# elasticdeeplearning/trainingjob-operator

Measured on AMD Instinct MI355X. Metric: tokens_per_sec_llama3_8b, higher is better.
Workload: dtype bf16; 1 GPU; model=llama3-8b, global_batch=4, seq_len=4096, parallelism=dp1, micro_batch=2, grad_accum=2, checkpoint_activations=False

## Files before the change

trainingjob_operator_amd/ops/hip/attention.hip:

```cpp

#include <hip/hip_runtime.h>
#include <hip/hip_bf16.h>
#include <cstdint>
#include <cstdlib>
#include <cstring>

typedef unsigned short u16;
typedef unsigned int u32;
typedef __attribute__((ext_vector_type(8))) __bf16 bf16x8;
typedef __attribute__((ext_vector_type(4))) float f32x4;

#define ATTN_BM 64
#define ATTN_BN 64
#define ATTN_D 128
#define ATTN_WAVES 4
__device__ __forceinline__ u16 attn_f2bf(float f) {
  __hip_bfloat16_raw r = __float2bfloat16(f);
  return r.x;
}

__device__ __forceinline__ float bf2f_(u16 b) {
  union { u32 u; float f; } c;
  c.u = ((u32)b) << 16;
  return c.f;
}

__device__ __forceinline__ int k_byte(int row, int col_elem) {
  return (row * ATTN_D * 2 + col_elem * 2) ^ ((row & 15) << 4);
}

#define VT_PITCH_B 144
__device__ __forceinline__ int vt_byte(int d, int kv) {
  const int m = d >> 3;
  return (d * VT_PITCH_B + kv * 2) ^
         ((((m & 7) | (((m >> 1) & 1) << 3))) << 4);
}

__device__ __forceinline__ int p_byte(int row, int col_elem) {
  return (row * ATTN_BN * 2 + col_elem * 2) ^ ((row & 7) << 4);
}


#define ATTN_SCHED_LEGACY 0
#define ATTN_SCHED_BALANCED 1

struct AttnBlock { int rank, head, batch; };

__host__ __device__ __forceinline__ AttnBlock attn_sched_block(
    unsigned id, unsigned n_row_blocks, unsigned n_heads, unsigned batch,
    int sched) {
  AttnBlock blk;
  if (sched == ATTN_SCHED_LEGACY) {
    const unsigned t = id / n_row_blocks;
    blk.rank = (int)(id - t * n_row_blocks);
    blk.batch = (int)(t / n_heads);
    blk.head = (int)(t - (unsigned)blk.batch * n_heads);
    return blk;
  }
  const unsigned M = n_heads * batch;
  const unsigned r = id / M;
  const unsigned w = id - r * M;
  const unsigned p = (M % 8 == 0) ? (w % 8) * (M / 8) + w / 8 : w;
  blk.rank = (int)r;
  blk.batch = (int)(p / n_heads);
  blk.head = (int)(p - (unsigned)blk.batch * n_heads);
  return blk;
}


#define ATTN_STRIPS_IDENTITY 0
#define ATTN_STRIPS_FOLD 1

struct AttnStrips { int kv0w, qt0; };

__host__ __device__ __forceinline__ AttnStrips attn_bwd_strips(
    int fold, int rank, int wid, int n_row_blocks) {
  AttnStrips s;
  if (fold == ATTN_STRIPS_IDENTITY) {
    s.kv0w = rank * 256 + wid * 32;
    s.qt0 = rank * 4;
    return s;
  }
  const int half = wid < 4 ? rank : 2 * n_row_blocks - 1 - rank;
  s.kv0w = half * 128 + (wid & 3) * 32;
  s.qt0 = rank * 2;
  return s;
}

__global__ __launch_bounds__(256) void attn_fwd_kernel(
    const u16* __restrict__ q, const u16* __restrict__ k,
    const u16* __restrict__ v, u16* __restrict__ out,
    float* __restrict__ lse,
    long q_sb, long q_sh, long q_ss,
    long k_sb, long k_sh, long k_ss,
    long v_sb, long v_sh, long v_ss,
    int n_heads, int S, float scale) {
  const int qb = blockIdx.x;
  const int h = blockIdx.y;
  const int b = blockIdx.z;
  const int wid = threadIdx.x >> 6;
  const int lane = threadIdx.x & 63;
  const int low = lane & 15;
  const int kg = lane >> 4;

  __shared__ u16 ldsK[ATTN_BN * ATTN_D];
  __shared__ u16 ldsV[ATTN_D * (VT_PITCH_B / 2) + 128];
  __shared__ u16 ldsP[ATTN_WAVES][16 * ATTN_BN];

  const u16* qbase = q + (long)b * q_sb + (long)h * q_sh
                     + (long)(qb * ATTN_BM) * q_ss;
  union { bf16x8 v; uint4 u; } qfrag[4];
#pragma unroll
  for (int ks = 0; ks < 4; ++ks) {
    qfrag[ks].u = *reinterpret_cast<const uint4*>(
        qbase + (long)(wid * 16 + low) * q_ss + ks * 32 + kg * 8);
  }

  float m_run[4], l_run[4];
  float oacc[8][4];
#pragma unroll
  for (int r = 0; r < 4; ++r) { m_run[r] = -INFINITY; l_run[r] = 0.f; }
#pragma unroll
  for (int ct = 0; ct < 8; ++ct)
#pragma unroll
    for (int r = 0; r < 4; ++r) oacc[ct][r] = 0.f;

  const u16* kbase = k + (long)b * k_sb + (long)h * k_sh;
  const u16* vbase = v + (long)b * v_sb + (long)h * v_sh;
  const int kv_end = (qb + 1) * ATTN_BM;
  char* ldsKb = reinterpret_cast<char*>(ldsK);
  char* ldsVb = reinterpret_cast<char*>(ldsV);
  char* ldsPb = reinterpret_cast<char*>(ldsP[wid]);

  for (int kv0 = 0; kv0 < kv_end; kv0 += ATTN_BN) {
#pragma unroll
    for (int t = 0; t < 4; ++t) {
      const int idx = t * 256 + threadIdx.x;
      const int r = idx >> 4;
      const int c8 = (idx & 15) * 8;
      *reinterpret_cast<uint4*>(&ldsKb[k_byte(r, c8)]) =
          *reinterpret_cast<const uint4*>(
              kbase + (long)(kv0 + r) * k_ss + c8);
      union { uint4 u; u16 h[8]; } vv;
      vv.u = *reinterpret_cast<const uint4*>(
          vbase + (long)(kv0 + r) * v_ss + c8);
#pragma unroll
      for (int j = 0; j < 8; ++j)
        *reinterpret_cast<u16*>(&ldsVb[vt_byte(c8 + j, r)]) = vv.h[j];
    }
    __syncthreads();

    f32x4 sacc[4];
#pragma unroll
    for (int ct = 0; ct < 4; ++ct) {
      f32x4 acc = {0.f, 0.f, 0.f, 0.f};
#pragma unroll
      for (int ks = 0; ks < 4; ++ks) {
        bf16x8 bfrag = *reinterpret_cast<const bf16x8*>(
            &ldsKb[k_byte(ct * 16 + low, ks * 32 + kg * 8)]);
        acc = __builtin_amdgcn_mfma_f32_16x16x32_bf16(qfrag[ks].v, bfrag,
                                                      acc, 0, 0, 0);
      }
      sacc[ct] = acc;
    }

    const int qrow0 = qb * ATTN_BM + wid * 16 + kg * 4;
    float mx[4], alpha[4], psum[4];
#pragma unroll
    for (int r = 0; r < 4; ++r) {
      mx[r] = -INFINITY;
#pragma unroll
      for (int ct = 0; ct < 4; ++ct) {
        const int col = kv0 + ct * 16 + low;
        float s = sacc[ct][r] * scale;
        if (col > qrow0 + r) s = -INFINITY;
        sacc[ct][r] = s;
        mx[r] = fmaxf(mx[r], s);
      }
#pragma unroll
      for (int off = 1; off < 16; off <<= 1)
        mx[r] = fmaxf(mx[r], __shfl_xor(mx[r], off, 64));
      const float mnew = fmaxf(m_run[r], mx[r]);
      alpha[r] = (m_run[r] == -INFINITY) ? 0.f : __expf(m_run[r] - mnew);
      m_run[r] = mnew;
      psum[r] = 0.f;
#pragma unroll
      for (int ct = 0; ct < 4; ++ct) {
        const float p = (sacc[ct][r] == -INFINITY)
                            ? 0.f : __expf(sacc[ct][r] - mnew);
        sacc[ct][r] = p;
        psum[r] += p;
        *reinterpret_cast<u16*>(
            &ldsPb[p_byte(kg * 4 + r, ct * 16 + low)]) = attn_f2bf(p);
      }
#pragma unroll
      for (int off = 1; off < 16; off <<= 1)
        psum[r] += __shfl_xor(psum[r], off, 64);
      l_run[r] = l_run[r] * alpha[r] + psum[r];
#pragma unroll
      for (int ct2 = 0; ct2 < 8; ++ct2) oacc[ct2][r] *= alpha[r];
    }
    __syncthreads();

#pragma unroll
    for (int ct2 = 0; ct2 < 8; ++ct2) {
      f32x4 acc = {oacc[ct2][0], oacc[ct2][1], oacc[ct2][2], oacc[ct2][3]};
#pragma unroll
      for (int ks2 = 0; ks2 < 2; ++ks2) {
        bf16x8 afrag = *reinterpret_cast<const bf16x8*>(
            &ldsPb[p_byte(low, ks2 * 32 + kg * 8)]);
        bf16x8 bfrag = *reinterpret_cast<const bf16x8*>(
            &ldsVb[vt_byte(ct2 * 16 + low, ks2 * 32 + kg * 8)]);
        acc = __builtin_amdgcn_mfma_f32_16x16x32_bf16(afrag, bfrag, acc,
                                                      0, 0, 0);
      }
#pragma unroll
      for (int r = 0; r < 4; ++r) oacc[ct2][r] = acc[r];
    }
    __syncthreads();
  }

  u16* obase = out + (((long)b * n_heads + h) * S + qb * ATTN_BM
                      + wid * 16) * ATTN_D;
#pragma unroll
  for (int r = 0; r < 4; ++r) {
    const float inv_l = 1.0f / l_run[r];
#pragma unroll
    for (int ct2 = 0; ct2 < 8; ++ct2) {
      obase[(long)(kg * 4 + r) * ATTN_D + ct2 * 16 + low] =
          attn_f2bf(oacc[ct2][r] * inv_l);
    }
  }
  if (low == 0) {
    float* lbase = lse + ((long)b * n_heads + h) * S + qb * ATTN_BM
                   + wid * 16 + kg * 4;
#pragma unroll
    for (int r = 0; r < 4; ++r) lbase[r] = m_run[r] + __logf(l_run[r]);
  }
}
// ... 1003 lines not shown
        qgp[i] += qstep;                                                    \
        __builtin_amdgcn_global_load_lds(                                   \
            (const u32*)dgp[i],                                             \
            (u32*)&lds[BUFI][DOOFF / 2 + (i * 512 + wu64 * 64) * 8],        \
            16, 0, 0);                                                      \
        dgp[i] += dostep;                                                   \
      }                                                                     \
      qtst[0] = *reinterpret_cast<const uint4*>(qtp[0]);                    \
      qtst[1] = *reinterpret_cast<const uint4*>(qtp[1]);                    \
      qtp[0] += qstep;                                                      \
      qtp[1] += qstep;                                                      \
      if (tid < 64)                                                         \
        *reinterpret_cast<float*>(&lds[BUFI][LSEOFF / 2 + tid * 2]) =       \
            lbase[(QT) * 64 + tid] * 1.4426950408889634f;                   \
      else if (tid < 128)                                                   \
        *reinterpret_cast<float*>(                                          \
            &lds[BUFI][DLTOFF / 2 + (tid - 64) * 2]) =                      \
            dbase[(QT) * 64 + tid - 64];                                    \
    }
#define BK_WRITE_QT(BUF)                                                    \
    {                                                                       \
      const int rp2_ = (tid >> 4) * 2;                                      \
      const int c8_ = (tid & 15) * 8;                                       \
      union { uint4 u4; u16 h[8]; } va_, vb_;                               \
      va_.u4 = qtst[0];                                                     \
      vb_.u4 = qtst[1];                                                     \
      _Pragma("unroll")                                                     \
      for (int j = 0; j < 8; ++j) {                                         \
        const u32 pair_ = (u32)va_.h[j] | ((u32)vb_.h[j] << 16);            \
        *reinterpret_cast<u32*>(&(BUF)[QTOFF + vt_byte(c8_ + j, rp2_)]) =   \
            pair_;                                                          \
      }                                                                     \
    }

    BK_STAGE_IN(0, qt0)
    BK_WRITE_QT(lds0)
    __syncthreads();

    int cur = 0;
    for (int qt = qt0; qt < qtn; ++qt) {
      const bool have_next = (qt + 1) < qtn;
      if (have_next) BK_STAGE_IN(cur ^ 1, qt + 1)

      char* qb_ = cur ? lds1 : lds0;
      char* dob = qb_ + DOOFF;
      char* qtb = qb_ + QTOFF;
      const float* lse2t = reinterpret_cast<const float*>(qb_ + LSEOFF);
      const float* dltt = reinterpret_cast<const float*>(qb_ + DLTOFF);
      const bool active = !CAUSAL || qt * 64 + 63 >= kv0w;
      const bool need_mask = CAUSAL && qt * 64 < kv0w + 32;

      union PF { bf16x8 v; unsigned u[4]; } pf[4];
      if (active) {
#pragma unroll
        for (int sub = 0; sub < 2; ++sub) {
          f32x16 s, dp;
#pragma unroll
          for (int r = 0; r < 16; ++r) { s[r] = 0.f; dp[r] = 0.f; }
#pragma unroll
          for (int kc = 0; kc < 8; ++kc) {
            bf16x8 a = *reinterpret_cast<const bf16x8*>(
                &qb_[k_byte(sub * 32 + low, kc * 16 + hi * 8)]);
            s = __builtin_amdgcn_mfma_f32_32x32x16_bf16(a, kf[kc].v, s,
                                                        0, 0, 0);
            bf16x8 a2 = *reinterpret_cast<const bf16x8*>(
                &dob[k_byte(sub * 32 + low, kc * 16 + hi * 8)]);
            dp = __builtin_amdgcn_mfma_f32_32x32x16_bf16(a2, vf[kc].v, dp,
                                                         0, 0, 0);
          }
#pragma unroll
          for (int r = 0; r < 16; ++r) {
            const int qr = (r & 3) + 8 * (r >> 2) + 4 * hi;
            float x = s[r] * scale2 - lse2t[sub * 32 + qr];
            if (need_mask && qt * 64 + sub * 32 + qr < kvrow) x = -1e30f;
            const float p = exp2_raw(x);
            s[r] = p * (dp[r] - dltt[sub * 32 + qr]) * scale;
          }
#pragma unroll
          for (int cc = 0; cc < 2; ++cc) {
            const int pb = cc * 8;
            unsigned a0 = cvt_pk_bf16(s[pb + 0], s[pb + 1]);
            unsigned b0 = cvt_pk_bf16(s[pb + 4], s[pb + 5]);
            unsigned a1 = cvt_pk_bf16(s[pb + 2], s[pb + 3]);
            unsigned b1 = cvt_pk_bf16(s[pb + 6], s[pb + 7]);
            auto r02 = __builtin_amdgcn_permlane32_swap(a0, b0, false, false);
            auto r13 = __builtin_amdgcn_permlane32_swap(a1, b1, false, false);
            PF f;
            f.u[0] = r02[0];
            f.u[1] = r13[0];
            f.u[2] = r02[1];
            f.u[3] = r13[1];
            pf[sub * 2 + cc] = f;
          }
        }
      }
      if (have_next) {
        char* nb = cur ? lds0 : lds1;
        BK_WRITE_QT(nb)
      }
      if (active) {
#pragma unroll
        for (int c = 0; c < 4; ++c) {
#pragma unroll
          for (int ds = 0; ds < 4; ++ds) {
            bf16x8 af = *reinterpret_cast<const bf16x8*>(
                &qtb[vt_byte(ds * 32 + low, c * 16 + hi * 8)]);
            dkacc[ds] = __builtin_amdgcn_mfma_f32_32x32x16_bf16(
                af, pf[c].v, dkacc[ds], 0, 0, 0);
          }
        }
      }
      __syncthreads();
      cur ^= 1;
    }
  }

  if (SPLIT) {
    float* wrow =
        ws + (((long)b * n_heads + blk.head) * S_kv + kvrow) * ATTN_D;
#pragma unroll
    for (int ds = 0; ds < 4; ++ds) {
#pragma unroll
      for (int g = 0; g < 4; ++g) {
        const int d0 = 8 * g + 4 * hi + 32 * ds;
        float4 wv;
        wv.x = dkacc[ds][4 * g + 0];
        wv.y = dkacc[ds][4 * g + 1];
        wv.z = dkacc[ds][4 * g + 2];
        wv.w = dkacc[ds][4 * g + 3];
        *reinterpret_cast<float4*>(wrow + d0) = wv;
      }
    }
    return;
  }
  u16* dkrow = dk + (long)b * dk_sb + (long)hkv * dk_sh + (long)kvrow * dk_ss;
#pragma unroll
  for (int ds = 0; ds < 4; ++ds) {
#pragma unroll
    for (int g = 0; g < 4; ++g) {
      const int d0 = 8 * g + 4 * hi + 32 * ds;
      const unsigned w0 = cvt_pk_bf16(dkacc[ds][4 * g + 0],
                                      dkacc[ds][4 * g + 1]);
      const unsigned w1 = cvt_pk_bf16(dkacc[ds][4 * g + 2],
                                      dkacc[ds][4 * g + 3]);
      uint2 wv;
      wv.x = w0;
      wv.y = w1;
      *reinterpret_cast<uint2*>(dkrow + d0) = wv;
    }
  }
}




struct AttnStride { long sb, sh, ss; };

static inline AttnStride attn_dense_stride(int n_heads, int S) {
  return {(long)n_heads * S * ATTN_D, (long)S * ATTN_D, (long)ATTN_D};
}

static void launch_delta(hipStream_t st, const void* out, const void* dout,
                         void* delta, AttnStride os, AttnStride dos,
                         int batch, int n_heads, int S) {
  hipLaunchKernelGGL(attn_delta_kernel, dim3(S / 16, n_heads, batch),
                     dim3(256), 0, st,
                     (const u16*)dout, (const u16*)out, (float*)delta,
                     dos.sb, dos.sh, dos.ss, os.sb, os.sh, os.ss,
                     n_heads, S);
}


__global__ __launch_bounds__(256) void attn_bwd_reduce_kernel(
    const float* __restrict__ ws_k, const float* __restrict__ ws_v,
    u16* __restrict__ dk, u16* __restrict__ dv,
    long dk_sb, long dk_sh, long dk_ss,
    long dv_sb, long dv_sh, long dv_ss,
    int n_heads, int n_kv_heads, int S, long n_rows) {
  const long row = (long)blockIdx.x * 16 + (threadIdx.x >> 4);
  if (row >= n_rows) return;
  const int sub = threadIdx.x & 15;
  const int gqa_group = n_heads / n_kv_heads;
  const long bh = row / S;
  const int s = (int)(row - bh * S);
  const long bi = bh / n_kv_heads;
  const int hkv = (int)(bh - bi * n_kv_heads);
  const bool is_v = blockIdx.y != 0;
  const float* src = (is_v ? ws_v : ws_k)
      + ((bi * n_heads + (long)hkv * gqa_group) * S + s) * ATTN_D + sub * 8;
  const long hstep = (long)S * ATTN_D;
  float4 a0 = reinterpret_cast<const float4*>(src)[0];
  float4 a1 = reinterpret_cast<const float4*>(src)[1];
  for (int g = 1; g < gqa_group; ++g) {
    const float4 p0 = reinterpret_cast<const float4*>(src + g * hstep)[0];
    const float4 p1 = reinterpret_cast<const float4*>(src + g * hstep)[1];
    a0.x += p0.x; a0.y += p0.y; a0.z += p0.z; a0.w += p0.w;
    a1.x += p1.x; a1.y += p1.y; a1.z += p1.z; a1.w += p1.w;
  }
  uint4 o;
  o.x = cvt_pk_bf16(a0.x, a0.y);
  o.y = cvt_pk_bf16(a0.z, a0.w);
  o.z = cvt_pk_bf16(a1.x, a1.y);
  o.w = cvt_pk_bf16(a1.z, a1.w);
  u16* dst = is_v
      ? dv + bi * dv_sb + (long)hkv * dv_sh + (long)s * dv_ss
      : dk + bi * dk_sb + (long)hkv * dk_sh + (long)s * dk_ss;
  *reinterpret_cast<uint4*>(dst + sub * 8) = o;
}

static inline bool attn_block_shape_ok(int batch, int n_heads,
                                       int n_kv_heads, int S) {
  return S > 0 && S % 256 == 0 && n_heads > 0 && batch > 0 &&
         n_kv_heads > 0 && n_heads % n_kv_heads == 0 &&
         attn_grid_ok(S, n_heads, batch);
}

#define ATTN_NUM_CUS 256
static bool attn_bwd_use_split(int batch, int n_heads, int n_kv_heads, int S,
                               bool causal) {
  const char* e = std::getenv("AITJ_ATTN_BWD_SPLIT");
  if (e && std::strcmp(e, "1") == 0) return true;
  if (!e || std::strcmp(e, "auto") != 0) return false;
  if (n_heads == n_kv_heads) return false;
  const long wgs = (long)batch * n_kv_heads * (S / 256);
  return wgs < (long)(causal ? 2 : 1) * ATTN_NUM_CUS;
}

static int attn_bwd_use_fold(int batch, int n_heads, int n_kv_heads, int S,
                             bool causal, bool split) {
  if (!causal) return ATTN_STRIPS_IDENTITY;
  const char* e = std::getenv("AITJ_ATTN_BWD_FOLD");
  if (e && std::strcmp(e, "0") == 0) return ATTN_STRIPS_IDENTITY;
  if (e && std::strcmp(e, "1") == 0) return ATTN_STRIPS_FOLD;
  const long wgs = (long)batch * (split ? n_heads : n_kv_heads) * (S / 256);
  return wgs <= ATTN_NUM_CUS ? ATTN_STRIPS_FOLD : ATTN_STRIPS_IDENTITY;
}

extern "C" int attn_bwd_strips_decode(int fold, int rank, int wid,
                                      int n_row_blocks, int* kv0w, int* qt0) {
  if (n_row_blocks <= 0 || rank < 0 || rank >= n_row_blocks || wid < 0 ||
      wid >= 8 || (fold != ATTN_STRIPS_IDENTITY && fold != ATTN_STRIPS_FOLD))
    return -1;
  const AttnStrips s = attn_bwd_strips(fold, rank, wid, n_row_blocks);
  *kv0w = s.kv0w;
  *qt0 = s.qt0;
  return 0;
}

extern "C" long attn_bwd_ws_bytes(int batch, int n_heads, int n_kv_heads,
                                  int S, int causal) {
  if (!attn_block_shape_ok(batch, n_heads, n_kv_heads, S)) return 0;
  if (!attn_bwd_use_split(batch, n_heads, n_kv_heads, S, causal != 0))
    return 0;
  return 2L * batch * n_heads * S * ATTN_D * (long)sizeof(float);
}

static inline bool attn_rect_shape_ok(int batch, int n_heads, int n_kv_heads,
                                      int S_q, int S_kv, bool causal) {
  return attn_block_shape_ok(batch, n_heads, n_kv_heads, S_q) &&
         attn_block_shape_ok(batch, n_heads, n_kv_heads, S_kv) &&
         !(causal && S_q != S_kv);
}

extern "C" long attn_bwd_ws_bytes_rect(int batch, int n_heads, int n_kv_heads,
                                       int S_q, int S_kv, int causal) {
  if (!attn_rect_shape_ok(batch, n_heads, n_kv_heads, S_q, S_kv, causal != 0))
    return 0;
  if (!attn_bwd_use_split(batch, n_heads, n_kv_heads, S_kv, causal != 0))
    return 0;
  return 2L * batch * n_heads * S_kv * ATTN_D * (long)sizeof(float);
}

template <bool CAUSAL>
static void launch_bwd_core(hipStream_t st, const void* q, const void* k,
                            const void* v, const void* dout,
                            const void* lse, const void* delta,
                            void* dq, void* dk, void* dv,
                            AttnStride qs, AttnStride ks, AttnStride vs,
                            AttnStride dos, AttnStride dqs, AttnStride dks,
                            AttnStride dvs, int batch, int n_heads,
                            int n_kv_heads, int S, int S_kv, float scale,
                            void* ws) {
  const int sched = attn_sched_mode();
  {
    dim3 grid((S / 256) * n_heads * batch), block(512);
    hipLaunchKernelGGL(attn_bwd_dq_kernel<CAUSAL>, grid, block, 0, st,
                       (const u16*)q, (const u16*)k, (const u16*)v,
                       (const u16*)dout, (const float*)lse,
                       (const float*)delta, (u16*)dq,
                       qs.sb, qs.sh, qs.ss, ks.sb, ks.sh, ks.ss,
                       vs.sb, vs.sh, vs.ss, dos.sb, dos.sh, dos.ss,
                       dqs.sb, dqs.sh, dqs.ss,
                       n_heads, n_heads / n_kv_heads, S, scale, batch, sched,
                       S_kv);
  }
  const int nrb = S_kv / 256;
  const bool split = ws != nullptr;
  float* ws_k = (float*)ws;
  float* ws_v = split ? ws_k + (long)batch * n_heads * S_kv * ATTN_D : nullptr;
  const int fold = attn_bwd_use_fold(batch, n_heads, n_kv_heads, S_kv, CAUSAL,
                                     split);
  dim3 grid(nrb * (split ? n_heads : n_kv_heads) * batch), block(512);
  auto dv_kernel = split ? attn_bwd_dv_kernel<CAUSAL, true>
                         : attn_bwd_dv_kernel<CAUSAL, false>;
  hipLaunchKernelGGL(dv_kernel, grid, block, 0, st,
                     (const u16*)q, (const u16*)k, (const u16*)dout,
                     (const float*)lse, (u16*)dv,
                     qs.sb, qs.sh, qs.ss, ks.sb, ks.sh, ks.ss,
                     dos.sb, dos.sh, dos.ss, dvs.sb, dvs.sh, dvs.ss,
                     n_heads, n_kv_heads, S, scale, ws_v, batch, sched, fold,
                     S_kv);
  auto dk_kernel = split ? attn_bwd_dk_kernel<CAUSAL, true>
                         : attn_bwd_dk_kernel<CAUSAL, false>;
  hipLaunchKernelGGL(dk_kernel, grid, block, 0, st,
                     (const u16*)q, (const u16*)k, (const u16*)v,
                     (const u16*)dout, (const float*)lse,
                     (const float*)delta, (u16*)dk,
                     qs.sb, qs.sh, qs.ss, ks.sb, ks.sh, ks.ss,
                     vs.sb, vs.sh, vs.ss, dos.sb, dos.sh, dos.ss,
                     dks.sb, dks.sh, dks.ss,
                     n_heads, n_kv_heads, S, scale, ws_k, batch, sched, fold,
                     S_kv);
  if (split) {
    const long n_rows = (long)batch * n_kv_heads * S_kv;
    hipLaunchKernelGGL(attn_bwd_reduce_kernel,
                       dim3((unsigned)((n_rows + 15) / 16), 2), dim3(256), 0,
                       st, (const float*)ws_k, (const float*)ws_v,
                       (u16*)dk, (u16*)dv, dks.sb, dks.sh, dks.ss,
                       dvs.sb, dvs.sh, dvs.ss, n_heads, n_kv_heads, S_kv,
                       n_rows);
  }
}

struct AttnBwdArgs {
  const void *q, *k, *v, *out, *dout, *lse;
  void *delta, *dq, *dk, *dv;
  AttnStride qs, ks, vs, os, dos, dqs, dks, dvs;
  int batch, n_heads, n_kv_heads, S;
  float scale;
  bool causal;
  bool with_delta;
  int S_kv = 0;
};

static long attn_bwd_need(const AttnBwdArgs& a) {
  if (a.S_kv == 0 || a.S_kv == a.S) {
    if (!attn_block_shape_ok(a.batch, a.n_heads, a.n_kv_heads, a.S)) return -1;
    return attn_bwd_ws_bytes(a.batch, a.n_heads, a.n_kv_heads, a.S, a.causal);
  }
  if (!attn_rect_shape_ok(a.batch, a.n_heads, a.n_kv_heads, a.S, a.S_kv,
                          a.causal))
    return -1;
  return attn_bwd_ws_bytes_rect(a.batch, a.n_heads, a.n_kv_heads, a.S, a.S_kv,
                                a.causal);
}

static int launch_bwd_ws(hipStream_t st, const AttnBwdArgs& a, void* ws,
                         long ws_bytes) {
  const long need = attn_bwd_need(a);
  if (need < 0) return -1;
  if (need > 0 && (ws == nullptr || ws_bytes < need)) return -2;
  if (need == 0) ws = nullptr;
  const int S_kv = a.S_kv ? a.S_kv : a.S;
  if (a.with_delta)
    launch_delta(st, a.out, a.dout, a.delta, a.os, a.dos, a.batch, a.n_heads,
                 a.S);
  if (a.causal)
    launch_bwd_core<true>(st, a.q, a.k, a.v, a.dout, a.lse, a.delta, a.dq,
                          a.dk, a.dv, a.qs, a.ks, a.vs, a.dos, a.dqs, a.dks,
                          a.dvs, a.batch, a.n_heads, a.n_kv_heads, a.S, S_kv,
                          a.scale, ws);
  else
    launch_bwd_core<false>(st, a.q, a.k, a.v, a.dout, a.lse, a.delta, a.dq,
                           a.dk, a.dv, a.qs, a.ks, a.vs, a.dos, a.dqs, a.dks,
                           a.dvs, a.batch, a.n_heads, a.n_kv_heads, a.S, S_kv,
                           a.scale, ws);
  return 0;
}

static int launch_bwd_transient(hipStream_t st, const AttnBwdArgs& a) {
  const long need = attn_bwd_need(a);
  if (need < 0) return -1;
  if (need == 0) return launch_bwd_ws(st, a, nullptr, 0);
  hipStreamCaptureStatus cs = hipStreamCaptureStatusNone;
  if (hipStreamIsCapturing(st, &cs) != hipSuccess ||
      cs != hipStreamCaptureStatusNone)
    return -3;
  void* ws = nullptr;
  if (hipMallocAsync(&ws, (size_t)need, st) != hipSuccess || !ws) return -4;
  const int rc = launch_bwd_ws(st, a, ws, need);
  if (hipFreeAsync(ws, st) != hipSuccess) return -5;
  return rc;
}

static AttnBwdArgs attn_bwd_dense_args(
    const void* q, const void* k, const void* v, const void* out,
    const void* dout, const void* lse, void* delta, void* dq, void* dk,
    void* dv, long q_sb, long q_sh, long q_ss, long k_sb, long k_sh,
    long k_ss, long v_sb, long v_sh, long v_ss, int batch, int n_heads,
    int n_kv_heads, int S, float scale) {
  const AttnStride dh = attn_dense_stride(n_heads, S);
  const AttnStride dkv = attn_dense_stride(n_kv_heads, S);
  return AttnBwdArgs{q, k, v, out, dout, lse, delta, dq, dk, dv,
                     {q_sb, q_sh, q_ss}, {k_sb, k_sh, k_ss},
                     {v_sb, v_sh, v_ss}, dh, dh, dh, dkv, dkv,
                     batch, n_heads, n_kv_heads, S, scale, true, true};
}

extern "C" int attn_bwd(void* stream, const void* q, const void* k,
                        const void* v, const void* out, const void* dout,
                        const void* lse, void* delta,
                        void* dq, void* dk, void* dv,
                        long q_sb, long q_sh, long q_ss,
                        long k_sb, long k_sh, long k_ss,
                        long v_sb, long v_sh, long v_ss,
                        int batch, int n_heads, int n_kv_heads, int S,
                        float scale) {
  return launch_bwd_transient(
      reinterpret_cast<hipStream_t>(stream),
      attn_bwd_dense_args(q, k, v, out, dout, lse, delta, dq, dk, dv,
                          q_sb, q_sh, q_ss, k_sb, k_sh, k_ss,
                          v_sb, v_sh, v_ss, batch, n_heads, n_kv_heads, S,
                          scale));
}

extern "C" int attn_bwd_ws(void* stream, const void* q, const void* k,
                           const void* v, const void* out, const void* dout,
                           const void* lse, void* delta,
                           void* dq, void* dk, void* dv,
                           long q_sb, long q_sh, long q_ss,
                           long k_sb, long k_sh, long k_ss,
                           long v_sb, long v_sh, long v_ss,
                           int batch, int n_heads, int n_kv_heads, int S,
                           float scale, void* ws, long ws_bytes) {
  return launch_bwd_ws(
      reinterpret_cast<hipStream_t>(stream),
      attn_bwd_dense_args(q, k, v, out, dout, lse, delta, dq, dk, dv,
                          q_sb, q_sh, q_ss, k_sb, k_sh, k_ss,
                          v_sb, v_sh, v_ss, batch, n_heads, n_kv_heads, S,
                          scale),
      ws, ws_bytes);
}

static bool attn_bwd_strided_args(
    AttnBwdArgs* a, const void* q, const void* k, const void* v,
    const void* out, const void* dout, const void* lse, void* delta,
    void* dq, void* dk, void* dv, const long* st, int batch, int n_heads,
    int n_kv_heads, int S, float scale) {
  if (!st || !attn_strides_ok(st, 24)) return false;
  auto tri = [st](int i) {
    return AttnStride{st[3 * i], st[3 * i + 1], st[3 * i + 2]};
  };
  *a = AttnBwdArgs{q, k, v, out, dout, lse, delta, dq, dk, dv,
                   tri(0), tri(1), tri(2), tri(3), tri(4), tri(5), tri(6),
                   tri(7), batch, n_heads, n_kv_heads, S, scale, true, true};
  return true;
}

extern "C" int attn_bwd_strided(void* stream, const void* q, const void* k,
                                const void* v, const void* out,
                                const void* dout, const void* lse,
                                void* delta, void* dq, void* dk, void* dv,
                                const long* st, int batch, int n_heads,
                                int n_kv_heads, int S, float scale) {
  AttnBwdArgs a;
  if (!attn_bwd_strided_args(&a, q, k, v, out, dout, lse, delta, dq, dk, dv,
                             st, batch, n_heads, n_kv_heads, S, scale))
    return -1;
  return launch_bwd_transient(reinterpret_cast<hipStream_t>(stream), a);
}

extern "C" int attn_bwd_strided_ws(void* stream, const void* q, const void* k,
                                   const void* v, const void* out,
                                   const void* dout, const void* lse,
                                   void* delta, void* dq, void* dk, void* dv,
// ... 455 lines not shown
```

trainingjob_operator_amd/ops/native.py:

```python
from __future__ import annotations

import ctypes
import os
import subprocess
from typing import Optional

_PKG_DIR = os.path.dirname(os.path.abspath(__file__))
LIB_PATH = os.path.join(_PKG_DIR, "libhipops.so")
SRC_PATH = os.path.join(_PKG_DIR, "hip", "ops.hip")
ATTN_SRC_PATH = os.path.join(_PKG_DIR, "hip", "attention.hip")

_lib: Optional[ctypes.CDLL] = None


class HipOpsUnavailable(RuntimeError):
    pass


def build_ops(verbose: bool = False) -> str:
    cmd = [
        "hipcc", "--offload-arch=gfx950", "-O3", "-std=c++17",
        "-shared", "-fPIC", SRC_PATH, ATTN_SRC_PATH, "-o", LIB_PATH,
    ]
    if verbose:
        print("+", " ".join(cmd))
    subprocess.run(cmd, check=True)
    return LIB_PATH


def _sig(fn, argtypes, restype=None):
    fn.argtypes = argtypes
    fn.restype = restype


def load(require: bool = True) -> Optional[ctypes.CDLL]:
    global _lib
    if _lib is not None:
        return _lib
    if not os.path.exists(LIB_PATH):
        if require:
            raise HipOpsUnavailable(
                f"{LIB_PATH} not built — run trainingjob_operator_amd.ops."
                "native.build_ops() (or __graft_entry__.build())")
        return None
    lib = ctypes.CDLL(LIB_PATH)
    vp, l, i, f = ctypes.c_void_p, ctypes.c_long, ctypes.c_int, ctypes.c_float
    _sig(lib.hipops_arch_check, [], i)
    _sig(lib.rmsnorm_fwd, [vp, vp, vp, vp, vp, vp, vp, l, i, f], i)
    _sig(lib.rmsnorm_bwd, [vp, vp, vp, vp, vp, vp, vp, vp, l, i], i)
    _sig(lib.rmsnorm_bwd_partials, [l, i], l)
    _sig(lib.rmsnorm_dw_reduce, [vp, vp, l, vp, i], i)
    _sig(lib.rope, [vp, vp, vp, vp, l, i, i, i, f], i)
    _sig(lib.rope_at, [vp, vp, vp, vp, l, i, i, i, f, i], i)
    _sig(lib.rope_at_dev, [vp, vp, vp, vp, l, i, i, i, f, vp], i)
    _sig(lib.rope_packed, [vp, vp, vp, vp, l, i, l, l, i, i, f], i)
    _sig(lib.rope_packed_at, [vp, vp, vp, vp, l, i, l, l, i, i, f, i, i, i],
         i)
    _sig(lib.gemv_bf16, [vp, vp, vp, vp, i, i, i], i)
    _sig(lib.gemv_swiglu, [vp, vp, vp, vp, i, i, i], i)
    _sig(lib.gemv_moe_swiglu, [vp, vp, vp, vp, vp, vp, i, i, i, i], i)
    _sig(lib.gemv_moe, [vp, vp, vp, vp, vp, i, i, i, i], i)
    _sig(lib.attn_decode, [vp, vp, vp, vp, vp, vp, vp,
                           i, i, i, i, i, f], i)
    _sig(lib.rope_cache, [vp, vp, vp, vp, vp, vp, vp, i, i, i, i, i], i)
    _sig(lib.swiglu_fwd, [vp, vp, vp, vp, l], i)
    _sig(lib.swiglu_bwd, [vp, vp, vp, vp, vp, vp, l], i)
    _sig(lib.swiglu_packed_fwd, [vp, vp, vp, l, i], i)
    _sig(lib.swiglu_packed_bwd, [vp, vp, vp, vp, l, i], i)
    _sig(lib.ce_fwd, [vp, vp, vp, vp, vp, l, i, i], i)
    _sig(lib.ce_bwd, [vp, vp, vp, vp, vp, vp, l, i, i], i)
    _sig(lib.l2normsq, [vp, vp, l, vp, i, vp], i)
    _sig(lib.rows_gather, [vp, vp, vp, vp, l, i], i)
    _sig(lib.rows_scatter, [vp, vp, vp, vp, l, i], i)
    _sig(lib.rows_scatter_add_f32, [vp, vp, vp, vp, l, i], i)
    _sig(lib.moe_combine, [vp, vp, vp, vp, vp, l, i, i], i)
    _sig(lib.moe_combine_bwd, [vp, vp, vp, vp, vp, vp, vp, l, i, i], i)
    _sig(lib.adamw_step, [vp, vp, vp, vp, vp, vp, vp, l,
                          f, f, f, f, f, f, f, f, f, vp], i)
    _sig(lib.adamw_step_bf16mom, [vp, vp, vp, vp, vp, vp, vp, l,
                                  f, f, f, f, f, f, f, f, f, vp], i)
    _sig(lib.mfma_probe, [vp, vp, vp, vp])
    _sig(lib.attn_fwd, [vp, vp, vp, vp, vp, vp,
                        l, l, l, l, l, l, l, l, l, i, i, i, i, f], i)
    _sig(lib.attn_fwd_v5, [vp, vp, vp, vp, vp, vp,
                           l, l, l, l, l, l, l, l, l, i, i, i, f], i)
    _sig(lib.attn_fwd_nw8, [vp, vp, vp, vp, vp, vp,
                            l, l, l, l, l, l, l, l, l, i, i, i, i, f], i)
    _sig(lib.attn_fwd_v7, [vp, vp, vp, vp, vp, vp,
                           l, l, l, l, l, l, l, l, l, i, i, i, i, f], i)
    _sig(lib.attn_bwd, [vp, vp, vp, vp, vp, vp, vp, vp, vp, vp, vp,
                        l, l, l, l, l, l, l, l, l, i, i, i, i, f], i)
    lp = ctypes.POINTER(ctypes.c_long)
    _sig(lib.attn_fwd_strided, [vp, vp, vp, vp, vp, vp, lp, i, i, i, i, f], i)
    _sig(lib.attn_bwd_strided, [vp, vp, vp, vp, vp, vp, vp, vp, vp, vp, vp,
                                lp, i, i, i, i, f], i)
    _sig(lib.attn_block_fwd, [vp, vp, vp, vp, vp, vp, lp,
                              i, i, i, i, f, i], i)
    _sig(lib.attn_delta, [vp, vp, vp, vp, lp, i, i, i], i)
    _sig(lib.attn_block_bwd, [vp, vp, vp, vp, vp, vp, vp, vp, vp, vp, lp,
                              i, i, i, i, f, i], i)
    _sig(lib.attn_merge, [vp, vp, vp, vp, vp, lp, i, i, i], i)
    _sig(lib.attn_bwd_ws_bytes, [i, i, i, i, i], l)
    _sig(lib.attn_bwd_ws, [vp, vp, vp, vp, vp, vp, vp, vp, vp, vp, vp,
                           l, l, l, l, l, l, l, l, l, i, i, i, i, f,
                           vp, l], i)
    _sig(lib.attn_bwd_strided_ws, [vp, vp, vp, vp, vp, vp, vp, vp, vp, vp,
                                   vp, lp, i, i, i, i, f, vp, l], i)
    _sig(lib.attn_block_bwd_ws, [vp, vp, vp, vp, vp, vp, vp, vp, vp, vp, lp,
                                 i, i, i, i, f, i, vp, l], i)
    _sig(lib.attn_block_fwd_rect, [vp, vp, vp, vp, vp, vp, lp,
                                   i, i, i, i, i, f, i], i)
    _sig(lib.attn_block_bwd_rect, [vp, vp, vp, vp, vp, vp, vp, vp, vp, vp, lp,
                                   i, i, i, i, i, f, i], i)
    _sig(lib.attn_block_bwd_rect_ws, [vp, vp, vp, vp, vp, vp, vp, vp, vp, vp,
                                      lp, i, i, i, i, i, f, i, vp, l], i)
    _sig(lib.attn_bwd_ws_bytes_rect, [i, i, i, i, i, i], l)
    ip = ctypes.POINTER(ctypes.c_int)
    _sig(lib.attn_sched_decode, [i, i, i, i, i, ip, ip, ip], i)
    _sig(lib.attn_bwd_strips_decode, [i, i, i, i, ip, ip], i)
    _sig(lib.mfma_probe32, [vp, vp, vp, vp])
    assert lib.hipops_arch_check() == 950
    _lib = lib
    return lib


def check_rc(rc: int, op: str, detail: str = "") -> None:
    if rc != 0:
        raise RuntimeError(
            f"hipops {op}: unsupported shape ({detail}) — the kernel "
            f"launcher refused to launch (rc={rc})")


def stride_array(*triples):
    flat = [int(x) for t in triples for x in t]
    assert len(flat) == 3 * len(triples)
    return (ctypes.c_long * len(flat))(*flat)


def available() -> bool:
    return os.path.exists(LIB_PATH)


def stream_ptr() -> ctypes.c_void_p:
    import torch
    return ctypes.c_void_p(torch.cuda.current_stream().cuda_stream)


def tr_probe_maps(device="cuda"):
    import torch
    lib = load()
    lib.tr_probe.argtypes = [ctypes.c_void_p, ctypes.c_void_p,
                             ctypes.c_int, ctypes.c_int]
    results = {}
    for mode in (0, 1, 2, 3):
        out = torch.empty(64, 4, dtype=torch.int16, device=device)
        lib.tr_probe(stream_ptr(), ctypes.c_void_p(out.data_ptr()), 0, mode)
        torch.cuda.synchronize()
        results[mode] = out.to(torch.int32).cpu() & 0xFFFF
    return results
```

Baseline: 20130 tokens/s.

## Add paired-wave causal dK backward kernel with LDS score exchange

Adds pair-mode backward kernels for causal attention. Each workgroup processes a folded pair of 128-row KV strips in two phases. The 8 waves split into two groups that each compute scores for half of the 64 query rows. The resulting P or dS tiles are exchanged through a small shared-memory buffer, so each wave accumulates only half of the head dimension. By default, pair mode is selected only for the dK kernel when the non-split grid fits within the CU count; dV keeps the fold scheme. The intent is to cut per-wave accumulator registers and duplicated MFMA work, at the cost of an extra LDS round trip and barrier per query tile.

```diff
diff --git a/trainingjob_operator_amd/ops/hip/attention.hip b/trainingjob_operator_amd/ops/hip/attention.hip
--- a/trainingjob_operator_amd/ops/hip/attention.hip
+++ b/trainingjob_operator_amd/ops/hip/attention.hip
@@ -85,6 +85,28 @@
   s.kv0w = half * 128 + (wid & 3) * 32;
   s.qt0 = rank * 2;
   return s;
+}
+
+
+#define ATTN_STRIPS_PAIR 2
+
+struct AttnPair { int kv0w, qt0, sub, ds0, peer; };
+
+__host__ __device__ __forceinline__ AttnPair attn_bwd_pair(
+    int rank, int phase, int wid, int n_row_blocks) {
+  AttnPair p;
+  const int hb = phase == 0 ? rank : 2 * n_row_blocks - 1 - rank;
+  p.kv0w = hb * 128 + (wid & 3) * 32;
+  p.qt0 = hb * 2;
+  p.sub = wid >> 2;
+  p.ds0 = (wid >> 2) * 2;
+  p.peer = wid ^ 4;
+  return p;
+}
+
+#define ATTN_PAIR_XCH_U4 (4 * 4 * 64)
+__host__ __device__ __forceinline__ int attn_pair_xch(int wid, int c) {
+  return ((wid & 3) * 4 + c) * 64;
 }
 
 __global__ __launch_bounds__(256) void attn_fwd_kernel(
@@ -1394,6 +1416,380 @@
 }
 
 
+__global__ __launch_bounds__(512) void attn_bwd_dv_pair_kernel(
+    const u16* __restrict__ q, const u16* __restrict__ k,
+    const u16* __restrict__ dout, const float* __restrict__ lse,
+    u16* __restrict__ dv,
+    long q_sb, long q_sh, long q_ss,
+    long k_sb, long k_sh, long k_ss,
+    long do_sb, long do_sh, long do_ss,
+    long dv_sb, long dv_sh, long dv_ss,
+    int n_heads, int n_kv_heads, int S, float scale, int batch, int sched) {
+  const int nrb = S / 256;
+  const AttnBlock blk = attn_sched_block(blockIdx.x, nrb, n_kv_heads, batch,
+                                         sched);
+  const int gqa_group = n_heads / n_kv_heads;
+  const int hkv = blk.head;
+  const int b = blk.batch;
+  const int tid = threadIdx.x;
+  const int lane = tid & 63;
+  const int low = lane & 31;
+  const int hi = lane >> 5;
+  const float scale2 = scale * 1.4426950408889634f;
+
+  __shared__ __attribute__((aligned(16))) u16 lds[2][BV_BUF_U16];
+  __shared__ __attribute__((aligned(16))) uint4 xch[ATTN_PAIR_XCH_U4];
+  char* lds0 = reinterpret_cast<char*>(&lds[0][0]);
+  char* lds1 = reinterpret_cast<char*>(&lds[1][0]);
+  const int DOTOFF = BV_Q_U16 * 2;
+  const int LSEOFF = (BV_Q_U16 + BV_DOT_U16) * 2;
+
+  const int qtn = S / 64;
+  const int wu64 = __builtin_amdgcn_readfirstlane(tid >> 6);
+  union F8 { bf16x8 v; uint4 u; u16 h[8]; };
+  uint4 dtst[2];
+
+#pragma unroll 1
+  for (int phase = 0; phase < 2; ++phase) {
+    const AttnPair pr = attn_bwd_pair(blk.rank, phase, wu64, nrb);
+    const int kv0w = pr.kv0w;
+    const int kvrow = kv0w + low;
+    const int sub = pr.sub;
+    const int aoff = pr.ds0 * 32 * VT_PITCH_B;
+
+    const u16* kptr =
+        k + (long)b * k_sb + (long)hkv * k_sh + (long)kvrow * k_ss;
+    F8 kf[8];
+#pragma unroll
+    for (int kc = 0; kc < 8; ++kc)
+      kf[kc].u = *reinterpret_cast<const uint4*>(kptr + kc * 16 + hi * 8);
+
+    f32x16 dvacc[2];
+#pragma unroll
+    for (int j = 0; j < 2; ++j)
+#pragma unroll
+      for (int r = 0; r < 16; ++r) dvacc[j][r] = 0.f;
+
+    const int qt0 = pr.qt0;
+
+    for (int g = 0; g < gqa_group; ++g) {
+      const int h = hkv * gqa_group + g;
+      const u16* qbase = q + (long)b * q_sb + (long)h * q_sh;
+      const u16* dobase = dout + (long)b * do_sb + (long)h * do_sh;
+      const float* lbase = lse + ((long)b * n_heads + h) * S;
+
+      const u16* qgp[2];
+      const u16* dtp[2];
+      {
+        const int idx0 = tid, idx1 = 512 + tid;
+        const int L0 = idx0 * 16, L1 = idx1 * 16;
+        const int r0 = L0 >> 8, r1 = L1 >> 8;
+        const int in0 = (((L0 & 255) ^ ((r0 & 15) << 4)) >> 1);
+        const int in1 = (((L1 & 255) ^ ((r1 & 15) << 4)) >> 1);
+        qgp[0] = qbase + (long)(qt0 * 64 + r0) * q_ss + in0;
+        qgp[1] = qbase + (long)(qt0 * 64 + r1) * q_ss + in1;
+        const int rp2 = (tid >> 4) * 2;
+        const int c8 = (tid & 15) * 8;
+        dtp[0] = dobase + (long)(qt0 * 64 + rp2) * do_ss + c8;
+        dtp[1] = dobase + (long)(qt0 * 64 + rp2 + 1) * do_ss + c8;
+      }
+      const long qstep = (long)64 * q_ss;
+      const long dostep = (long)64 * do_ss;
+
+      BV_STAGE_IN(0, qt0)
+      BV_WRITE_DOT(lds0)
+      __syncthreads();
+
+      int cur = 0;
+      for (int qt = qt0; qt < qtn; ++qt) {
+        const bool have_next = (qt + 1) < qtn;
+        if (have_next) BV_STAGE_IN(cur ^ 1, qt + 1)
+
+        char* qb_ = cur ? lds1 : lds0;
+        char* dob = qb_ + DOTOFF;
+        const float* lse2t = reinterpret_cast<const float*>(qb_ + LSEOFF);
+        const bool active = qt * 64 + 63 >= kv0w;
+        const bool need_mask = qt * 64 < kv0w + 32;
+
+        union PF { bf16x8 v; unsigned u[4]; uint4 q4; } pf[4];
+        if (active) {
+          f32x16 s;
+#pragma unroll
+          for (int r = 0; r < 16; ++r) s[r] = 0.f;
+#pragma unroll
+          for (int kc = 0; kc < 8; ++kc) {
+            bf16x8 a = *reinterpret_cast<const bf16x8*>(
+                &qb_[k_byte(sub * 32 + low, kc * 16 + hi * 8)]);
+            s = __builtin_amdgcn_mfma_f32_32x32x16_bf16(a, kf[kc].v, s,
+                                                        0, 0, 0);
+          }
+#pragma unroll
+          for (int r = 0; r < 16; ++r) {
+            const int qr = (r & 3) + 8 * (r >> 2) + 4 * hi;
+            float x = s[r] * scale2 - lse2t[sub * 32 + qr];
+            if (need_mask && qt * 64 + sub * 32 + qr < kvrow) x = -1e30f;
+            s[r] = exp2_raw(x);
+          }
+#pragma unroll
+          for (int cc = 0; cc < 2; ++cc) {
+            const int pb = cc * 8;
+            unsigned a0 = cvt_pk_bf16(s[pb + 0], s[pb + 1]);
+            unsigned b0 = cvt_pk_bf16(s[pb + 4], s[pb + 5]);
+            unsigned a1 = cvt_pk_bf16(s[pb + 2], s[pb + 3]);
+            unsigned b1 = cvt_pk_bf16(s[pb + 6], s[pb + 7]);
+            auto r02 = __builtin_amdgcn_permlane32_swap(a0, b0, false, false);
+            auto r13 = __builtin_amdgcn_permlane32_swap(a1, b1, false, false);
+            PF f;
+            f.u[0] = r02[0];
+            f.u[1] = r13[0];
+            f.u[2] = r02[1];
+            f.u[3] = r13[1];
+            xch[attn_pair_xch(wu64, sub * 2 + cc) + lane] = f.q4;
+          }
+        }
+        v7_barrier();
+        if (active) {
+#pragma unroll
+          for (int c = 0; c < 4; ++c)
+            pf[c].q4 = xch[attn_pair_xch(wu64, c) + lane];
+        }
+        if (have_next) {
+          char* nb = cur ? lds0 : lds1;
+          BV_WRITE_DOT(nb)
+        }
+        if (active) {
+#pragma unroll
+          for (int c = 0; c < 4; ++c) {
+#pragma unroll
+            for (int j = 0; j < 2; ++j) {
+              bf16x8 af = *reinterpret_cast<const bf16x8*>(
+                  &dob[aoff + vt_byte(j * 32 + low, c * 16 + hi * 8)]);
+              dvacc[j] = __builtin_amdgcn_mfma_f32_32x32x16_bf16(
+                  af, pf[c].v, dvacc[j], 0, 0, 0);
+            }
+          }
+        }
+        __syncthreads();
+        cur ^= 1;
+      }
+    }
+
+    u16* dvrow =
+        dv + (long)b * dv_sb + (long)hkv * dv_sh + (long)kvrow * dv_ss;
+#pragma unroll
+    for (int j = 0; j < 2; ++j) {
+#pragma unroll
+      for (int g = 0; g < 4; ++g) {
+        const int d0 = 8 * g + 4 * hi + 32 * (pr.ds0 + j);
+        const unsigned w0 = cvt_pk_bf16(dvacc[j][4 * g + 0],
+                                        dvacc[j][4 * g + 1]);
+        const unsigned w1 = cvt_pk_bf16(dvacc[j][4 * g + 2],
+                                        dvacc[j][4 * g + 3]);
+        uint2 wv;
+        wv.x = w0;
+        wv.y = w1;
+        *reinterpret_cast<uint2*>(dvrow + d0) = wv;
+      }
+    }
+  }
+}
+
+__global__ __launch_bounds__(512) void attn_bwd_dk_pair_kernel(
+    const u16* __restrict__ q, const u16* __restrict__ k,
+    const u16* __restrict__ v, const u16* __restrict__ dout,
+    const float* __restrict__ lse, const float* __restrict__ delta,
+    u16* __restrict__ dk,
+    long q_sb, long q_sh, long q_ss,
+    long k_sb, long k_sh, long k_ss,
+    long v_sb, long v_sh, long v_ss,
+    long do_sb, long do_sh, long do_ss,
+    long dk_sb, long dk_sh, long dk_ss,
+    int n_heads, int n_kv_heads, int S, float scale, int batch, int sched) {
+  const int nrb = S / 256;
+  const AttnBlock blk = attn_sched_block(blockIdx.x, nrb, n_kv_heads, batch,
+                                         sched);
+  const int gqa_group = n_heads / n_kv_heads;
+  const int hkv = blk.head;
+  const int b = blk.batch;
+  const int tid = threadIdx.x;
+  const int lane = tid & 63;
+  const int low = lane & 31;
+  const int hi = lane >> 5;
+  const float scale2 = scale * 1.4426950408889634f;
+
+  __shared__ __attribute__((aligned(16))) u16 lds[2][BK_BUF_U16];
+  __shared__ __attribute__((aligned(16))) uint4 xch[ATTN_PAIR_XCH_U4];
+  char* lds0 = reinterpret_cast<char*>(&lds[0][0]);
+  char* lds1 = reinterpret_cast<char*>(&lds[1][0]);
+  const int DOOFF = BK_Q_U16 * 2;
+  const int QTOFF = (BK_Q_U16 + BK_DO_U16) * 2;
+  const int LSEOFF = (BK_Q_U16 + BK_DO_U16 + BK_QT_U16) * 2;
+  const int DLTOFF = LSEOFF + BK_LSE_U16 * 2;
+
+  const int qtn = S / 64;
+  const int wu64 = __builtin_amdgcn_readfirstlane(tid >> 6);
+  union F8 { bf16x8 v; uint4 u; u16 h[8]; };
+  uint4 qtst[2];
+
+#pragma unroll 1
+  for (int phase = 0; phase < 2; ++phase) {
+    const AttnPair pr = attn_bwd_pair(blk.rank, phase, wu64, nrb);
+    const int kv0w = pr.kv0w;
+    const int kvrow = kv0w + low;
+    const int sub = pr.sub;
+    const int aoff = pr.ds0 * 32 * VT_PITCH_B;
+
+    const u16* kptr =
+        k + (long)b * k_sb + (long)hkv * k_sh + (long)kvrow * k_ss;
+    const u16* vptr =
+        v + (long)b * v_sb + (long)hkv * v_sh + (long)kvrow * v_ss;
+    F8 kf[8], vf[8];
+#pragma unroll
+    for (int kc = 0; kc < 8; ++kc) {
+      kf[kc].u = *reinterpret_cast<const uint4*>(kptr + kc * 16 + hi * 8);
+      vf[kc].u = *reinterpret_cast<const uint4*>(vptr + kc * 16 + hi * 8);
+    }
+
+    f32x16 dkacc[2];
+#pragma unroll
+    for (int j = 0; j < 2; ++j)
+#pragma unroll
+      for (int r = 0; r < 16; ++r) dkacc[j][r] = 0.f;
+
+    const int qt0 = pr.qt0;
+
+    for (int g = 0; g < gqa_group; ++g) {
+      const int h = hkv * gqa_group + g;
+      const u16* qbase = q + (long)b * q_sb + (long)h * q_sh;
+      const u16* dobase = dout + (long)b * do_sb + (long)h * do_sh;
+      const float* lbase = lse + ((long)b * n_heads + h) * S;
+      const float* dbase = delta + ((long)b * n_heads + h) * S;
+
+      const u16* qgp[2];
+      const u16* dgp[2];
+      const u16* qtp[2];
+      {
+        const int idx0 = tid, idx1 = 512 + tid;
+        const int L0 = idx0 * 16, L1 = idx1 * 16;
+        const int r0 = L0 >> 8, r1 = L1 >> 8;
+        const int in0 = (((L0 & 255) ^ ((r0 & 15) << 4)) >> 1);
+        const int in1 = (((L1 & 255) ^ ((r1 & 15) << 4)) >> 1);
+        qgp[0] = qbase + (long)(qt0 * 64 + r0) * q_ss + in0;
+        qgp[1] = qbase + (long)(qt0 * 64 + r1) * q_ss + in1;
+        dgp[0] = dobase + (long)(qt0 * 64 + r0) * do_ss + in0;
+        dgp[1] = dobase + (long)(qt0 * 64 + r1) * do_ss + in1;
+        const int rp2 = (tid >> 4) * 2;
+        const int c8 = (tid & 15) * 8;
+        qtp[0] = qbase + (long)(qt0 * 64 + rp2) * q_ss + c8;
+        qtp[1] = qbase + (long)(qt0 * 64 + rp2 + 1) * q_ss + c8;
+      }
+      const long qstep = (long)64 * q_ss;
+      const long dostep = (long)64 * do_ss;
+
+      BK_STAGE_IN(0, qt0)
+      BK_WRITE_QT(lds0)
+      __syncthreads();
+
+      int cur = 0;
+      for (int qt = qt0; qt < qtn; ++qt) {
+        const bool have_next = (qt + 1) < qtn;
+        if (have_next) BK_STAGE_IN(cur ^ 1, qt + 1)
+
+        char* qb_ = cur ? lds1 : lds0;
+        char* dob = qb_ + DOOFF;
+        char* qtb = qb_ + QTOFF;
+        const float* lse2t = reinterpret_cast<const float*>(qb_ + LSEOFF);
+        const float* dltt = reinterpret_cast<const float*>(qb_ + DLTOFF);
+        const bool active = qt * 64 + 63 >= kv0w;
+        const bool need_mask = qt * 64 < kv0w + 32;
+
+        union PF { bf16x8 v; unsigned u[4]; uint4 q4; } pf[4];
+        if (active) {
+          f32x16 s, dp;
+#pragma unroll
+          for (int r = 0; r < 16; ++r) { s[r] = 0.f; dp[r] = 0.f; }
+#pragma unroll
+          for (int kc = 0; kc < 8; ++kc) {
+            bf16x8 a = *reinterpret_cast<const bf16x8*>(
+                &qb_[k_byte(sub * 32 + low, kc * 16 + hi * 8)]);
+            s = __builtin_amdgcn_mfma_f32_32x32x16_bf16(a, kf[kc].v, s,
+                                                        0, 0, 0);
+            bf16x8 a2 = *reinterpret_cast<const bf16x8*>(
+                &dob[k_byte(sub * 32 + low, kc * 16 + hi * 8)]);
+            dp = __builtin_amdgcn_mfma_f32_32x32x16_bf16(a2, vf[kc].v, dp,
+                                                         0, 0, 0);
+          }
+#pragma unroll
+          for (int r = 0; r < 16; ++r) {
+            const int qr = (r & 3) + 8 * (r >> 2) + 4 * hi;
+            float x = s[r] * scale2 - lse2t[sub * 32 + qr];
+            if (need_mask && qt * 64 + sub * 32 + qr < kvrow) x = -1e30f;
+            const float p = exp2_raw(x);
+            s[r] = p * (dp[r] - dltt[sub * 32 + qr]) * scale;
+          }
+#pragma unroll
+          for (int cc = 0; cc < 2; ++cc) {
+            const int pb = cc * 8;
+            unsigned a0 = cvt_pk_bf16(s[pb + 0], s[pb + 1]);
+            unsigned b0 = cvt_pk_bf16(s[pb + 4], s[pb + 5]);
+            unsigned a1 = cvt_pk_bf16(s[pb + 2], s[pb + 3]);
+            unsigned b1 = cvt_pk_bf16(s[pb + 6], s[pb + 7]);
+            auto r02 = __builtin_amdgcn_permlane32_swap(a0, b0, false, false);
+            auto r13 = __builtin_amdgcn_permlane32_swap(a1, b1, false, false);
+            PF f;
+            f.u[0] = r02[0];
+            f.u[1] = r13[0];
+            f.u[2] = r02[1];
+            f.u[3] = r13[1];
+            xch[attn_pair_xch(wu64, sub * 2 + cc) + lane] = f.q4;
+          }
+        }
+        v7_barrier();
+        if (active) {
+#pragma unroll
+          for (int c = 0; c < 4; ++c)
+            pf[c].q4 = xch[attn_pair_xch(wu64, c) + lane];
+        }
+        if (have_next) {
+          char* nb = cur ? lds0 : lds1;
+          BK_WRITE_QT(nb)
+        }
+        if (active) {
+#pragma unroll
+          for (int c = 0; c < 4; ++c) {
+#pragma unroll
+            for (int j = 0; j < 2; ++j) {
+              bf16x8 af = *reinterpret_cast<const bf16x8*>(
+                  &qtb[aoff + vt_byte(j * 32 + low, c * 16 + hi * 8)]);
+              dkacc[j] = __builtin_amdgcn_mfma_f32_32x32x16_bf16(
+                  af, pf[c].v, dkacc[j], 0, 0, 0);
+            }
+          }
+        }
+        __syncthreads();
+        cur ^= 1;
+      }
+    }
+
+    u16* dkrow =
+        dk + (long)b * dk_sb + (long)hkv * dk_sh + (long)kvrow * dk_ss;
+#pragma unroll
+    for (int j = 0; j < 2; ++j) {
+#pragma unroll
+      for (int g = 0; g < 4; ++g) {
+        const int d0 = 8 * g + 4 * hi + 32 * (pr.ds0 + j);
+        const unsigned w0 = cvt_pk_bf16(dkacc[j][4 * g + 0],
+                                        dkacc[j][4 * g + 1]);
+        const unsigned w1 = cvt_pk_bf16(dkacc[j][4 * g + 2],
+                                        dkacc[j][4 * g + 3]);
+        uint2 wv;
+        wv.x = w0;
+        wv.y = w1;
+        *reinterpret_cast<uint2*>(dkrow + d0) = wv;
+      }
+    }
+  }
+}
 
 
 struct AttnStride { long sb, sh, ss; };
@@ -1468,14 +1864,41 @@
   return wgs < (long)(causal ? 2 : 1) * ATTN_NUM_CUS;
 }
 
+#define ATTN_BWD_DV 0
+#define ATTN_BWD_DK 1
 static int attn_bwd_use_fold(int batch, int n_heads, int n_kv_heads, int S,
-                             bool causal, bool split) {
+                             bool causal, bool split, int kernel) {
   if (!causal) return ATTN_STRIPS_IDENTITY;
   const char* e = std::getenv("AITJ_ATTN_BWD_FOLD");
   if (e && std::strcmp(e, "0") == 0) return ATTN_STRIPS_IDENTITY;
   if (e && std::strcmp(e, "1") == 0) return ATTN_STRIPS_FOLD;
+  if (e && std::strcmp(e, "2") == 0 && !split) return ATTN_STRIPS_PAIR;
   const long wgs = (long)batch * (split ? n_heads : n_kv_heads) * (S / 256);
-  return wgs <= ATTN_NUM_CUS ? ATTN_STRIPS_FOLD : ATTN_STRIPS_IDENTITY;
+  if (wgs > ATTN_NUM_CUS) return ATTN_STRIPS_IDENTITY;
+  if (split || kernel != ATTN_BWD_DK) return ATTN_STRIPS_FOLD;
+  return ATTN_STRIPS_PAIR;
+}
+
+extern "C" int attn_bwd_fold_mode(int batch, int n_heads, int n_kv_heads,
+                                  int S, int causal, int split, int kernel) {
+  return attn_bwd_use_fold(batch, n_heads, n_kv_heads, S, causal != 0,
+                           split != 0, kernel);
+}
+
+extern "C" int attn_bwd_pair_decode(int rank, int phase, int wid,
+                                    int n_row_blocks, int* kv0w, int* qt0,
+                                    int* sub, int* ds0, int* ds1, int* peer) {
+  if (n_row_blocks <= 0 || rank < 0 || rank >= n_row_blocks || wid < 0 ||
+      wid >= 8 || phase < 0 || phase > 1)
+    return -1;
+  const AttnPair p = attn_bwd_pair(rank, phase, wid, n_row_blocks);
+  *kv0w = p.kv0w;
+  *qt0 = p.qt0;
+  *sub = p.sub;
+  *ds0 = p.ds0;
+  *ds1 = p.ds0 + 2;
+  *peer = p.peer;
+  return 0;
 }
 
 extern "C" int attn_bwd_strips_decode(int fold, int rank, int wid,
@@ -1540,29 +1963,51 @@
   const bool split = ws != nullptr;
   float* ws_k = (float*)ws;
   float* ws_v = split ? ws_k + (long)batch * n_heads * S_kv * ATTN_D : nullptr;
-  const int fold = attn_bwd_use_fold(batch, n_heads, n_kv_heads, S_kv, CAUSAL,
-                                     split);
+  const int fold_v = attn_bwd_use_fold(batch, n_heads, n_kv_heads, S_kv,
+                                       CAUSAL, split, ATTN_BWD_DV);
+  const int fold_k = attn_bwd_use_fold(batch, n_heads, n_kv_heads, S_kv,
+                                       CAUSAL, split, ATTN_BWD_DK);
   dim3 grid(nrb * (split ? n_heads : n_kv_heads) * batch), block(512);
-  auto dv_kernel = split ? attn_bwd_dv_kernel<CAUSAL, true>
-                         : attn_bwd_dv_kernel<CAUSAL, false>;
-  hipLaunchKernelGGL(dv_kernel, grid, block, 0, st,
-                     (const u16*)q, (const u16*)k, (const u16*)dout,
-                     (const float*)lse, (u16*)dv,
-                     qs.sb, qs.sh, qs.ss, ks.sb, ks.sh, ks.ss,
-                     dos.sb, dos.sh, dos.ss, dvs.sb, dvs.sh, dvs.ss,
-                     n_heads, n_kv_heads, S, scale, ws_v, batch, sched, fold,
-                     S_kv);
-  auto dk_kernel = split ? attn_bwd_dk_kernel<CAUSAL, true>
-                         : attn_bwd_dk_kernel<CAUSAL, false>;
-  hipLaunchKernelGGL(dk_kernel, grid, block, 0, st,
-                     (const u16*)q, (const u16*)k, (const u16*)v,
-                     (const u16*)dout, (const float*)lse,
-                     (const float*)delta, (u16*)dk,
-                     qs.sb, qs.sh, qs.ss, ks.sb, ks.sh, ks.ss,
-                     vs.sb, vs.sh, vs.ss, dos.sb, dos.sh, dos.ss,
-                     dks.sb, dks.sh, dks.ss,
-                     n_heads, n_kv_heads, S, scale, ws_k, batch, sched, fold,
-                     S_kv);
+  if (fold_v == ATTN_STRIPS_PAIR) {
+    hipLaunchKernelGGL(attn_bwd_dv_pair_kernel, grid, block, 0, st,
+                       (const u16*)q, (const u16*)k, (const u16*)dout,
+                       (const float*)lse, (u16*)dv,
+                       qs.sb, qs.sh, qs.ss, ks.sb, ks.sh, ks.ss,
+                       dos.sb, dos.sh, dos.ss, dvs.sb, dvs.sh, dvs.ss,
+                       n_heads, n_kv_heads, S, scale, batch, sched);
+  } else {
+    auto dv_kernel = split ? attn_bwd_dv_kernel<CAUSAL, true>
+                           : attn_bwd_dv_kernel<CAUSAL, false>;
+    hipLaunchKernelGGL(dv_kernel, grid, block, 0, st,
+                       (const u16*)q, (const u16*)k, (const u16*)dout,
+                       (const float*)lse, (u16*)dv,
+                       qs.sb, qs.sh, qs.ss, ks.sb, ks.sh, ks.ss,
+                       dos.sb, dos.sh, dos.ss, dvs.sb, dvs.sh, dvs.ss,
+                       n_heads, n_kv_heads, S, scale, ws_v, batch, sched,
+                       fold_v, S_kv);
+  }
+  if (fold_k == ATTN_STRIPS_PAIR) {
+    hipLaunchKernelGGL(attn_bwd_dk_pair_kernel, grid, block, 0, st,
+                       (const u16*)q, (const u16*)k, (const u16*)v,
+                       (const u16*)dout, (const float*)lse,
+                       (const float*)delta, (u16*)dk,
+                       qs.sb, qs.sh, qs.ss, ks.sb, ks.sh, ks.ss,
+                       vs.sb, vs.sh, vs.ss, dos.sb, dos.sh, dos.ss,
+                       dks.sb, dks.sh, dks.ss,
+                       n_heads, n_kv_heads, S, scale, batch, sched);
+  } else {
+    auto dk_kernel = split ? attn_bwd_dk_kernel<CAUSAL, true>
+                           : attn_bwd_dk_kernel<CAUSAL, false>;
+    hipLaunchKernelGGL(dk_kernel, grid, block, 0, st,
+                       (const u16*)q, (const u16*)k, (const u16*)v,
+                       (const u16*)dout, (const float*)lse,
+                       (const float*)delta, (u16*)dk,
+                       qs.sb, qs.sh, qs.ss, ks.sb, ks.sh, ks.ss,
+                       vs.sb, vs.sh, vs.ss, dos.sb, dos.sh, dos.ss,
+                       dks.sb, dks.sh, dks.ss,
+                       n_heads, n_kv_heads, S, scale, ws_k, batch, sched,
+                       fold_k, S_kv);
+  }
   if (split) {
     const long n_rows = (long)batch * n_kv_heads * S_kv;
     hipLaunchKernelGGL(attn_bwd_reduce_kernel,
diff --git a/trainingjob_operator_amd/ops/native.py b/trainingjob_operator_amd/ops/native.py
--- a/trainingjob_operator_amd/ops/native.py
+++ b/trainingjob_operator_amd/ops/native.py
@@ -118,6 +118,8 @@
     ip = ctypes.POINTER(ctypes.c_int)
     _sig(lib.attn_sched_decode, [i, i, i, i, i, ip, ip, ip], i)
     _sig(lib.attn_bwd_strips_decode, [i, i, i, i, ip, ip], i)
+    _sig(lib.attn_bwd_pair_decode, [i, i, i, i, ip, ip, ip, ip, ip, ip], i)
+    _sig(lib.attn_bwd_fold_mode, [i, i, i, i, i, i, i], i)
     _sig(lib.mfma_probe32, [vp, vp, vp, vp])
     assert lib.hipops_arch_check() == 950
     _lib = lib
```

Measured after the change: 20510 tokens/s, median of 6. +1.9%, better.
